# HKUST-KnowComp/DualMessagePassing

Measured on AMD Instinct MI355X. Metric: (pattern,graph) pairs/sec DMPNN fwd+bwd hid=128, higher is better.
Workload: dtype f32

## Files before the change

dualmessagepassing_amd/csrc/dmp_nodechain.hip:

```cpp
#include "dmp_mfma_common.h"

namespace dmp {
__device__ int llvm_struct_buffer_load_i32(i32x4 rsrc, int vindex, int voffset, int soffset, int aux) __asm("llvm.amdgcn.struct.buffer.load.i32");
__device__ void llvm_struct_buffer_store_i32(int data, i32x4 rsrc, int vindex, int voffset, int soffset, int aux) __asm("llvm.amdgcn.struct.buffer.store.i32");
namespace {

constexpr int kChainThreads = 512;
constexpr int kChainRows = 128;
constexpr int kChainStrideD = 68;
constexpr int kChainPlane = kChainRows * kChainStrideD;
constexpr int kChainImageBytes = 3 * kChainPlane * 4;
constexpr int kChainPanelBytes = 3 * 128 * 128 * 2;
constexpr int kChainChunkBytes = kChainPanelBytes / 4;
constexpr int kChainLdsBytes = kChainImageBytes + 2 * kChainChunkBytes + kChainRows * 4;
constexpr int kChainMaxPanels = 12;

__device__ __forceinline__ float sbuf_load1(srsrc_t r, int row, uint32_t col_bytes) {
  return __int_as_float(llvm_struct_buffer_load_i32(r, row, (int)col_bytes, 0, 0));
}
__device__ __forceinline__ void sbuf_store1(float v, srsrc_t r, int row, uint32_t col_bytes) {
  llvm_struct_buffer_store_i32(__float_as_int(v), r, row, (int)col_bytes, 0, 0);
}

struct PackArgs {
  const float *W[kChainMaxPanels];
  int64_t ld[kChainMaxPanels];
  int transposed[kChainMaxPanels];
  uint32_t *out;
};
__global__ __launch_bounds__(256) void chain_pack_k(PackArgs p) {
  const int item = (int)blockIdx.x * 256 + (int)threadIdx.x;
  const int lane = item & 63, cb = (item >> 6) & 3, g = item >> 8;
  const int li = lane & 31, h = lane >> 5;
  const float *W = nullptr;
  int64_t ld = 0;
  int tr = 0;
#pragma unroll
  for (int j = 0; j < kChainMaxPanels; ++j)
    if (j == (int)blockIdx.y) { W = p.W[j]; ld = p.ld[j]; tr = p.transposed[j]; }
  const int k0 = 64 * h + 8 * g, c = 32 * cb + li;
  float w[8];
#pragma unroll
  for (int j = 0; j < 8; ++j) w[j] = tr ? W[(int64_t)c * ld + k0 + j] : W[(int64_t)(k0 + j) * ld + c];
  Split8 s;
  split8(make_float4(w[0], w[1], w[2], w[3]), make_float4(w[4], w[5], w[6], w[7]), s);
  uint32_t *o = p.out + (size_t)blockIdx.y * (kChainPanelBytes / 4) + (size_t)g * 3072 + cb * 256 + lane * 4;
  *reinterpret_cast<uint4 *>(o) = make_uint4(s.hi.u[0], s.hi.u[1], s.hi.u[2], s.hi.u[3]);
  *reinterpret_cast<uint4 *>(o + 1024) = make_uint4(s.mid.u[0], s.mid.u[1], s.mid.u[2], s.mid.u[3]);
  *reinterpret_cast<uint4 *>(o + 2048) = make_uint4(s.lo.u[0], s.lo.u[1], s.lo.u[2], s.lo.u[3]);
}

struct ChainArgs {
  const float *A0, *A1, *A2;
  int64_t lda0, lda1, lda2;
  const float *X; int64_t ldx;
  const float *Res; int64_t ldres;
  const float *bias1, *bias2;
  float *O0, *O1, *O2, *O3;
  int64_t ldo0, ldo1, ldo2, ldo3;
  float *partial, *partialA;
  const uint32_t *panels;
  int npanels;
  const int32_t *slot; const int32_t *num_tiles;
  int64_t rows;
  float slope;
};

template <bool BWD, bool FULL>
__global__ __launch_bounds__(kChainThreads) void node_chain_k(ChainArgs p) {
  extern __shared__ __attribute__((aligned(256))) unsigned char lds[];
  uint32_t *Aimg = reinterpret_cast<uint32_t *>(lds);
  unsigned char *Pb = lds + kChainImageBytes;
  int *ids_s = reinterpret_cast<int *>(lds + kChainImageBytes + 2 * kChainChunkBytes);

  const int t = threadIdx.x;
  const int wave = __builtin_amdgcn_readfirstlane(t >> 6);
  const int lane = t & 63, li = lane & 31, h = lane >> 5;
  const int rt = wave >> 1, ch = wave & 1;
  const int q = t & 31, r0 = t >> 5;
  const float slope = __builtin_bit_cast(float, __builtin_amdgcn_readfirstlane(__builtin_bit_cast(int, p.slope)));
  const bool has_res = p.Res != nullptr;
  const int NC = __builtin_amdgcn_readfirstlane(p.npanels) * 4;
  constexpr bool full = FULL;

  const int ntiles = __builtin_amdgcn_readfirstlane(*p.num_tiles);
  const int chunk = (ntiles + (int)gridDim.x - 1) / (int)gridDim.x;
  const int lo = (int)blockIdx.x * chunk;
  const int hi = lo + chunk < ntiles ? lo + chunk : ntiles;
  if (hi <= lo) {
    if (BWD && t < 128) { p.partial[(int64_t)blockIdx.x * 128 + t] = 0.f; p.partialA[(int64_t)blockIdx.x * 128 + t] = 0.f; }
    return;
  }
  const rsrc_t rs_slot = make_rsrc(p.slot, (uint32_t)hi * (kSub * 4u));
  const rsrc_t rs_pan = make_rsrc(p.panels, (uint32_t)NC * (uint32_t)kChainChunkBytes);
  const srsrc_t rs_A0 = make_srsrc(p.A0, p.lda0, p.rows), rs_A1 = make_srsrc(p.A1, p.lda1, p.rows), rs_A2 = make_srsrc(p.A2, p.lda2, p.rows);
  const srsrc_t rs_X = make_srsrc(p.X, p.X ? p.ldx : (int64_t)128, p.X ? p.rows : 0);
  const srsrc_t rs_Res = make_srsrc(p.Res, has_res ? p.ldres : (int64_t)128, has_res ? p.rows : 0);
  const srsrc_t rs_O0 = make_srsrc(p.O0, p.ldo0, p.rows), rs_O1 = make_srsrc(p.O1, p.ldo1, p.rows), rs_O2 = make_srsrc(p.O2, p.ldo2, p.rows);
  const srsrc_t rs_O3 = make_srsrc(p.O3, p.O3 ? p.ldo3 : (int64_t)128, p.O3 ? p.rows : 0);

  int ids[8];
  float4 pre[8];
  auto load_ids = [&](int tile0) {
#pragma unroll
    for (int m = 0; m < 8; ++m) {
      const int idx = tile0 * kSub + r0 + 16 * m;
      const int v = (int)__builtin_amdgcn_raw_buffer_load_b32(rs_slot, idx * 4, 0, 0);
      ids[m] = idx < hi * kSub ? v : -1;
    }
  };
  auto load_rows = [&](srsrc_t rs) {
#pragma unroll
    for (int m = 0; m < 8; ++m) pre[m] = sbuf_load4(rs, ids[m], (uint32_t)q * 16u);
  };
  float4 csA = make_float4(0.f, 0.f, 0.f, 0.f);
  auto stage = [&](bool first) {
#pragma unroll
    for (int m = 0; m < 8; ++m) {
      const int row = r0 + 16 * m;
      if (BWD && first) { csA.x += pre[m].x; csA.y += pre[m].y; csA.z += pre[m].z; csA.w += pre[m].w; }
      uint2 ph, pm, pl;
      split_pair(pre[m].x, pre[m].y, ph.x, pm.x, pl.x);
      split_pair(pre[m].z, pre[m].w, ph.y, pm.y, pl.y);
      uint32_t *d = Aimg + row * kChainStrideD + q * 2;
      *reinterpret_cast<uint2 *>(d) = ph;
      *reinterpret_cast<uint2 *>(d + kChainPlane) = pm;
      *reinterpret_cast<uint2 *>(d + 2 * kChainPlane) = pl;
      if (first && q == 0) ids_s[row] = ids[m];
    }
  };

  f32x16 acc[2];
  auto zero_acc = [&]() {
#pragma unroll
    for (int r = 0; r < 16; ++r) { acc[0][r] = 0.f; acc[1][r] = 0.f; }
  };
  auto product = [&](int pidx) {
#pragma unroll
    for (int cc = 0; cc < 4; ++cc) {
      const int c = 4 * pidx + cc;
      const int nc = c + 1 == NC ? 0 : c + 1;
      uint4 pc[3];
#pragma unroll
      for (int i = 0; i < 3; ++i) {
        const u32x4 v = __builtin_amdgcn_raw_buffer_load_b128(rs_pan, (i * kChainThreads + t) * 16, nc * kChainChunkBytes, 0);
        pc[i] = make_uint4(v.x, v.y, v.z, v.w);
      }
      const unsigned char *pb = Pb + (cc & 1) * kChainChunkBytes;
      const uint32_t *ar = Aimg + (32 * rt + li) * kChainStrideD + 32 * h;
#pragma unroll
      for (int gl = 0; gl < 2; ++gl) {
        const int g = 2 * cc + gl;
        Split8 a;
        a.hi.v = *reinterpret_cast<const bf16x8 *>(ar + 4 * g);
        a.mid.v = *reinterpret_cast<const bf16x8 *>(ar + kChainPlane + 4 * g);
        a.lo.v = *reinterpret_cast<const bf16x8 *>(ar + 2 * kChainPlane + 4 * g);
#pragma unroll
        for (int cbl = 0; cbl < 2; ++cbl) {
          const unsigned char *bq = pb + gl * 12288 + (2 * ch + cbl) * 1024 + lane * 16;
          Split8 b;
          b.hi.v = *reinterpret_cast<const bf16x8 *>(bq);
          b.mid.v = *reinterpret_cast<const bf16x8 *>(bq + 4096);
          b.lo.v = *reinterpret_cast<const bf16x8 *>(bq + 8192);
          acc[cbl] = mfma_x6(a, b, acc[cbl]);
        }
      }
      uint4 *pw = reinterpret_cast<uint4 *>(Pb + ((cc + 1) & 1) * kChainChunkBytes);
#pragma unroll
      for (int i = 0; i < 3; ++i) pw[i * kChainThreads + t] = pc[i];
      lds_barrier();
    }
  };
  int rid[16];
  auto store_acc = [&](srsrc_t rs) {
#pragma unroll
    for (int cb = 0; cb < 2; ++cb)
#pragma unroll
      for (int r = 0; r < 16; ++r) sbuf_store1(acc[cb][r], rs, rid[r], (uint32_t)(64 * ch + 32 * cb + li) * 4u);
  };
  auto acc_to_image = [&]() {
#pragma unroll
    for (int cb = 0; cb < 2; ++cb)
#pragma unroll
      for (int i = 0; i < 8; ++i) {
        const float va = acc[cb][2 * i], vb = acc[cb][2 * i + 1];
        const float got = __shfl_xor((li & 1) ? va : vb, 1, 64);
        const float f0 = (li & 1) ? got : va, f1 = (li & 1) ? vb : got;
        const int r = 2 * i + (li & 1);
        const int row = 32 * rt + (r & 3) + 8 * (r >> 2) + 4 * h;
        uint32_t ph, pm, pl;
        split_pair(f0, f1, ph, pm, pl);
        uint32_t *d = Aimg + row * kChainStrideD + 32 * ch + 16 * cb + (li >> 1);
        d[0] = ph; d[kChainPlane] = pm; d[2 * kChainPlane] = pl;
      }
  };
  float colsum[2] = {0.f, 0.f};

  load_ids(lo);
  load_rows(rs_A0);
  {
    uint4 *pw = reinterpret_cast<uint4 *>(Pb);
#pragma unroll
    for (int i = 0; i < 3; ++i) {
      const u32x4 v = __builtin_amdgcn_raw_buffer_load_b128(rs_pan, (i * kChainThreads + t) * 16, 0, 0);
      pw[i * kChainThreads + t] = make_uint4(v.x, v.y, v.z, v.w);
    }
  }
  for (int g0 = lo; g0 < hi; g0 += 4) {
    stage(true);
    lds_barrier();
#pragma unroll
    for (int qd = 0; qd < 4; ++qd) {
      const int4 v = *reinterpret_cast<const int4 *>(&ids_s[32 * rt + 8 * qd + 4 * h]);
      rid[4 * qd] = v.x; rid[4 * qd + 1] = v.y; rid[4 * qd + 2] = v.z; rid[4 * qd + 3] = v.w;
    }
    if (!BWD) {
      load_rows(rs_A1);
      zero_acc(); product(0); store_acc(rs_O0);
      zero_acc(); product(1); store_acc(rs_O1);
      zero_acc(); product(2);
      stage(false); lds_barrier();
      load_rows(rs_A2);
      product(3);
      stage(false); lds_barrier();
      load_ids(g0 + 4);
      product(4);
      load_rows(rs_A0);
#pragma unroll
      for (int cb = 0; cb < 2; ++cb) {
        const float b = p.bias1[64 * ch + 32 * cb + li];
#pragma unroll
        for (int r = 0; r < 16; ++r) acc[cb][r] = act_fwd(acc[cb][r] + b, slope);
      }
      float res[2][16];
#pragma unroll
      for (int cb = 0; cb < 2; ++cb)
#pragma unroll
        for (int r = 0; r < 16; ++r) res[cb][r] = sbuf_load1(rs_Res, rid[r], (uint32_t)(64 * ch + 32 * cb + li) * 4u);
      store_acc(rs_O2);
      acc_to_image();
      lds_barrier();
      zero_acc(); product(5);
#pragma unroll
      for (int cb = 0; cb < 2; ++cb) {
        const float b = p.bias2[64 * ch + 32 * cb + li];
#pragma unroll
        for (int r = 0; r < 16; ++r) acc[cb][r] = res[cb][r] + (acc[cb][r] + b);
      }
      store_acc(rs_O3);
    } else {
      float hv[2][16];
#pragma unroll
      for (int cb = 0; cb < 2; ++cb)
#pragma unroll
        for (int r = 0; r < 16; ++r) hv[cb][r] = sbuf_load1(rs_X, rid[r], (uint32_t)(64 * ch + 32 * cb + li) * 4u);
      zero_acc(); product(0);
      if (full) load_rows(rs_A1);
      else load_ids(g0 + 4);
#pragma unroll
      for (int cb = 0; cb < 2; ++cb)
#pragma unroll
        for (int r = 0; r < 16; ++r) {
          acc[cb][r] = act_bwd(hv[cb][r], acc[cb][r], slope);
          colsum[cb] += acc[cb][r];
        }
      store_acc(rs_O0);
      acc_to_image();
      lds_barrier();
      zero_acc(); product(1);
      if (!full) load_rows(rs_A0);
      store_acc(rs_O1);
      zero_acc(); product(2); store_acc(rs_O2);
      if (full) {
        zero_acc(); product(3);
        stage(false); lds_barrier();
        load_rows(rs_A2);
        product(4);
        stage(false); lds_barrier();
        load_ids(g0 + 4);
        float res[2][16];
#pragma unroll
        for (int cb = 0; cb < 2; ++cb)
#pragma unroll
          for (int r = 0; r < 16; ++r) res[cb][r] = sbuf_load1(rs_Res, rid[r], (uint32_t)(64 * ch + 32 * cb + li) * 4u);
        product(5);
        load_rows(rs_A0);
#pragma unroll
        for (int cb = 0; cb < 2; ++cb)
#pragma unroll
          for (int r = 0; r < 16; ++r) acc[cb][r] = res[cb][r] + acc[cb][r];
        store_acc(rs_O3);
      }
    }
  }
  if (BWD) {
    float *red = reinterpret_cast<float *>(Pb);
    float *redA = red + 4 * 128;
#pragma unroll
    for (int cb = 0; cb < 2; ++cb) {
      const float s = colsum[cb] + __shfl_xor(colsum[cb], 32, 64);
      if (h == 0) red[rt * 128 + 64 * ch + 32 * cb + li] = s;
    }
    *reinterpret_cast<float4 *>(&redA[r0 * 128 + q * 4]) = csA;
    lds_barrier();
    if (t < 128) {
      float s = red[t];
#pragma unroll
      for (int w = 1; w < 4; ++w) s += red[w * 128 + t];
      p.partial[(int64_t)blockIdx.x * 128 + t] = s;
      float sa = redA[t];
#pragma unroll
      for (int w = 1; w < 16; ++w) sa += redA[w * 128 + t];
      p.partialA[(int64_t)blockIdx.x * 128 + t] = sa;
    }
  }
}

inline unsigned chain_blocks(int64_t tiles_bound) {
  const int64_t want = (tiles_bound + 3) / 4;
  return (unsigned)(want < 1 ? 1 : (want > 256 ? 256 : want));
}

constexpr int kMaxDevicesC = 64;
template <bool BWD, bool FULL>
inline bool chain_lds_ready() {
  static bool done[kMaxDevicesC] = {};
  int dev = 0;
  if (hipGetDevice(&dev) != hipSuccess || dev < 0 || dev >= kMaxDevicesC) dev = 0;
  if (done[dev]) return true;
  const hipError_t e = hipFuncSetAttribute(reinterpret_cast<const void *>(&node_chain_k<BWD, FULL>), hipFuncAttributeMaxDynamicSharedMemorySize, kChainLdsBytes);
  if (e != hipSuccess) { set_last_hip_error(e); return false; }
  done[dev] = true;
  return true;
}

inline bool chain_rows_ok(const float *a, int64_t ld, int64_t rows) {
  return a && ld >= 128 && ld % 4 == 0 && aligned16(a) && stride_ok(ld) && fits4g(rows, ld);
}

}
}

using namespace dmp;

extern "C" {

int64_t dmp_node_chain_blocks(int64_t tiles_bound) { return (int64_t)chain_blocks(tiles_bound); }
int64_t dmp_node_chain_panel_words(void) { return kChainPanelBytes / 4; }

int dmp_node_chain_pack(const dmp_chain_panel *panels, int num_panels, uint32_t *out, void *stream) {
  if (!panels || !out || num_panels < 1 || num_panels > kChainMaxPanels || !aligned16(out)) return DMP_ERR_BAD_ARG;
  PackArgs a{};
  for (int j = 0; j < num_panels; ++j) {
    if (!panels[j].W || panels[j].ld < 128) return DMP_ERR_BAD_ARG;
    a.W[j] = panels[j].W; a.ld[j] = panels[j].ld; a.transposed[j] = panels[j].transposed ? 1 : 0;
  }
  a.out = out;
  chain_pack_k<<<dim3(8, (unsigned)num_panels), 256, 0, (hipStream_t)stream>>>(a);
  return check_launch();
}

int dmp_node_chain_fwd(const float *x, int64_t ldx, const float *S, int64_t lds, const uint32_t *panels, const float *bn, const float *b2,
                       int residual, float slope, const int32_t *slot, const int32_t *num_tiles, int64_t tiles_bound, int64_t rows, int H,
                       float *H1n, int64_t ldh, float *P, int64_t ldp, float *xn, int64_t ldxn, void *stream) {
  if (H != 128 || g_exact_fp32) return DMP_ERR_UNSUPPORTED;
  if (rows < 0 || tiles_bound < 0) return DMP_ERR_BAD_ARG;
  if (!slope_ok(slope)) return DMP_ERR_UNSUPPORTED;
  if (rows == 0 || tiles_bound == 0) return DMP_OK;
  if (!panels || !bn || !b2 || !slot || !num_tiles || !aligned16(panels)) return DMP_ERR_BAD_ARG;
  if (!x || !S || !H1n || !P || !xn || ldx < H || lds < 2 * H || ldh < H || ldp < 2 * H || ldxn < H) return DMP_ERR_BAD_ARG;
  if (!chain_rows_ok(x, ldx, rows) || !chain_rows_ok(S, lds, rows) || !chain_rows_ok(H1n, ldh, rows) || !chain_rows_ok(P, ldp, rows) ||
      !chain_rows_ok(xn, ldxn, rows) || rows >= ((int64_t)1 << 30) || tiles_bound * kSub * 4 >= ((int64_t)1 << 32) - 8192)
    return DMP_ERR_UNSUPPORTED;
  if (!chain_lds_ready<false, true>()) return DMP_ERR_HIP;
  ChainArgs a{};
  a.A0 = x; a.lda0 = ldx; a.A1 = S; a.lda1 = lds; a.A2 = S + H; a.lda2 = lds;
  a.Res = residual ? x : nullptr; a.ldres = ldx; a.bias1 = bn; a.bias2 = b2;
  a.O0 = P; a.ldo0 = ldp; a.O1 = P + H; a.ldo1 = ldp; a.O2 = H1n; a.ldo2 = ldh; a.O3 = xn; a.ldo3 = ldxn;
  a.panels = panels; a.npanels = 6; a.slot = slot; a.num_tiles = num_tiles; a.rows = rows; a.slope = slope;
  node_chain_k<false, true><<<chain_blocks(tiles_bound), kChainThreads, kChainLdsBytes, (hipStream_t)stream>>>(a);
  return check_launch();
}

int dmp_node_chain_bwd(const float *dxn, int64_t ldd, const float *H1n, int64_t ldh, const float *dP, int64_t ldp, const uint32_t *panels,
                       int residual, float slope, const int32_t *slot, const int32_t *num_tiles, int64_t tiles_bound, int64_t rows, int H,
                       float *dPn, int64_t ldn, float *dS, int64_t lds, float *dx, int64_t ldx, float *partial, float *partial_rows,
                       void *stream) {
  if (H != 128 || g_exact_fp32) return DMP_ERR_UNSUPPORTED;
  if (rows < 0 || tiles_bound < 0) return DMP_ERR_BAD_ARG;
  if (!slope_ok(slope)) return DMP_ERR_UNSUPPORTED;
  if (!partial || !partial_rows) return DMP_ERR_BAD_ARG;
  hipStream_t st = (hipStream_t)stream;
  if (rows == 0 || tiles_bound == 0) {
    const size_t bytes = sizeof(float) * 128 * (size_t)chain_blocks(tiles_bound);
    if (hipMemsetAsync(partial, 0, bytes, st) != hipSuccess || hipMemsetAsync(partial_rows, 0, bytes, st) != hipSuccess) return DMP_ERR_HIP;
    return DMP_OK;
  }
  if (!panels || !slot || !num_tiles || !aligned16(panels)) return DMP_ERR_BAD_ARG;
  if (!dxn || !H1n || !dPn || !dS || ldd < H || ldh < H || ldn < H || lds < 2 * H || (dx && (!dP || ldp < 2 * H || ldx < H))) return DMP_ERR_BAD_ARG;
  if (!chain_rows_ok(dxn, ldd, rows) || !chain_rows_ok(H1n, ldh, rows) || !chain_rows_ok(dPn, ldn, rows) || !chain_rows_ok(dS, lds, rows) ||
      (dx && (!chain_rows_ok(dP, ldp, rows) || !chain_rows_ok(dx, ldx, rows))) || rows >= ((int64_t)1 << 30) ||
      tiles_bound * kSub * 4 >= ((int64_t)1 << 32) - 8192)
    return DMP_ERR_UNSUPPORTED;
  if (!(dx ? chain_lds_ready<true, true>() : chain_lds_ready<true, false>())) return DMP_ERR_HIP;
  ChainArgs a{};
  a.A0 = dxn; a.lda0 = ldd;
  a.A1 = dx ? dP : dxn; a.lda1 = dx ? ldp : ldd; a.A2 = dx ? dP + H : dxn; a.lda2 = a.lda1;
  a.X = H1n; a.ldx = ldh; a.Res = (dx && residual) ? dxn : nullptr; a.ldres = ldd;
  a.O0 = dPn; a.ldo0 = ldn; a.O1 = dS; a.ldo1 = lds; a.O2 = dS + H; a.ldo2 = lds; a.O3 = dx; a.ldo3 = ldx;
  a.partial = partial; a.partialA = partial_rows;
  a.panels = panels; a.npanels = dx ? 6 : 3; a.slot = slot; a.num_tiles = num_tiles; a.rows = rows; a.slope = slope;
  if (dx) node_chain_k<true, true><<<chain_blocks(tiles_bound), kChainThreads, kChainLdsBytes, st>>>(a);
  else node_chain_k<true, false><<<chain_blocks(tiles_bound), kChainThreads, kChainLdsBytes, st>>>(a);
  return check_launch();
}

}
```

Before: 489,600.

## Stream weight panels directly to LDS and overlap output stores with next product

Panel chunks are now fetched with buffer-load-to-LDS instead of going through registers and then being written to shared memory. Each GEMM product's output stores are deferred into the first chunk iteration of the following product, so global stores overlap MFMA work, with hand-tuned vmcnt waits. The LDS layout is reordered so the panel buffers come first and the activation image offset is made opaque to the compiler. This cuts register pressure and VGPR-to-LDS traffic, but depends on fragile manual waitcnt counts that could race if the store count assumption is wrong.

Result: no change. 494,200, median of 6 (+0.9%).

```diff
diff --git a/dualmessagepassing_amd/csrc/dmp_nodechain.hip b/dualmessagepassing_amd/csrc/dmp_nodechain.hip
--- a/dualmessagepassing_amd/csrc/dmp_nodechain.hip
+++ b/dualmessagepassing_amd/csrc/dmp_nodechain.hip
@@ -69,9 +69,11 @@
 template <bool BWD, bool FULL>
 __global__ __launch_bounds__(kChainThreads) void node_chain_k(ChainArgs p) {
   extern __shared__ __attribute__((aligned(256))) unsigned char lds[];
-  uint32_t *Aimg = reinterpret_cast<uint32_t *>(lds);
-  unsigned char *Pb = lds + kChainImageBytes;
-  int *ids_s = reinterpret_cast<int *>(lds + kChainImageBytes + 2 * kChainChunkBytes);
+  unsigned char *Pb = lds;
+  int *ids_s = reinterpret_cast<int *>(lds + 2 * kChainChunkBytes);
+  int img_at = 2 * kChainChunkBytes + kChainRows * 4;
+  asm("" : "+v"(img_at));
+  uint32_t *Aimg = reinterpret_cast<uint32_t *>(lds + img_at);
 
   const int t = threadIdx.x;
   const int wave = __builtin_amdgcn_readfirstlane(t >> 6);
@@ -135,17 +137,27 @@
 #pragma unroll
     for (int r = 0; r < 16; ++r) { acc[0][r] = 0.f; acc[1][r] = 0.f; }
   };
-  auto product = [&](int pidx) {
+  int rid[16];
+  auto store_acc = [&](srsrc_t rs) {
+#pragma unroll
+    for (int cb = 0; cb < 2; ++cb)
+#pragma unroll
+      for (int r = 0; r < 16; ++r) sbuf_store1(acc[cb][r], rs, rid[r], (uint32_t)(64 * ch + 32 * cb + li) * 4u);
+  };
+  auto request_quarter = [&](int nc, int b) {
+#pragma unroll
+    for (int i = 0; i < 3; ++i)
+      __builtin_amdgcn_raw_ptr_buffer_load_lds(rs_pan, (__attribute__((address_space(3))) void *)(Pb + b * kChainChunkBytes + i * (kChainThreads * 16) + wave * 1024),
+                                               16, (i * kChainThreads + t) * 16, nc * kChainChunkBytes, 0, 0);
+  };
+  auto product = [&](int pidx, const srsrc_t *out) {
 #pragma unroll
     for (int cc = 0; cc < 4; ++cc) {
       const int c = 4 * pidx + cc;
-      const int nc = c + 1 == NC ? 0 : c + 1;
-      uint4 pc[3];
-#pragma unroll
-      for (int i = 0; i < 3; ++i) {
-        const u32x4 v = __builtin_amdgcn_raw_buffer_load_b128(rs_pan, (i * kChainThreads + t) * 16, nc * kChainChunkBytes, 0);
-        pc[i] = make_uint4(v.x, v.y, v.z, v.w);
-      }
+      request_quarter(c + 1 == NC ? 0 : c + 1, (cc + 1) & 1);
+      __builtin_amdgcn_sched_barrier(0);
+      const bool stores = cc == 0 && out != nullptr;
+      if (stores) { store_acc(*out); zero_acc(); }
       const unsigned char *pb = Pb + (cc & 1) * kChainChunkBytes;
       const uint32_t *ar = Aimg + (32 * rt + li) * kChainStrideD + 32 * h;
 #pragma unroll
@@ -165,18 +177,11 @@
           acc[cbl] = mfma_x6(a, b, acc[cbl]);
         }
       }
-      uint4 *pw = reinterpret_cast<uint4 *>(Pb + ((cc + 1) & 1) * kChainChunkBytes);
-#pragma unroll
-      for (int i = 0; i < 3; ++i) pw[i * kChainThreads + t] = pc[i];
+      __builtin_amdgcn_sched_barrier(0);
+      if (stores) asm volatile("s_waitcnt vmcnt(32)" ::: "memory");
+      else asm volatile("s_waitcnt vmcnt(0)" ::: "memory");
       lds_barrier();
     }
-  };
-  int rid[16];
-  auto store_acc = [&](srsrc_t rs) {
-#pragma unroll
-    for (int cb = 0; cb < 2; ++cb)
-#pragma unroll
-      for (int r = 0; r < 16; ++r) sbuf_store1(acc[cb][r], rs, rid[r], (uint32_t)(64 * ch + 32 * cb + li) * 4u);
   };
   auto acc_to_image = [&]() {
 #pragma unroll
@@ -196,16 +201,10 @@
   };
   float colsum[2] = {0.f, 0.f};
 
+  request_quarter(0, 0);
   load_ids(lo);
   load_rows(rs_A0);
-  {
-    uint4 *pw = reinterpret_cast<uint4 *>(Pb);
-#pragma unroll
-    for (int i = 0; i < 3; ++i) {
-      const u32x4 v = __builtin_amdgcn_raw_buffer_load_b128(rs_pan, (i * kChainThreads + t) * 16, 0, 0);
-      pw[i * kChainThreads + t] = make_uint4(v.x, v.y, v.z, v.w);
-    }
-  }
+  asm volatile("s_waitcnt vmcnt(0)" ::: "memory");
   for (int g0 = lo; g0 < hi; g0 += 4) {
     stage(true);
     lds_barrier();
@@ -216,15 +215,15 @@
     }
     if (!BWD) {
       load_rows(rs_A1);
-      zero_acc(); product(0); store_acc(rs_O0);
-      zero_acc(); product(1); store_acc(rs_O1);
-      zero_acc(); product(2);
+      zero_acc(); product(0, nullptr);
+      product(1, &rs_O0);
+      product(2, &rs_O1);
       stage(false); lds_barrier();
       load_rows(rs_A2);
-      product(3);
+      product(3, nullptr);
       stage(false); lds_barrier();
       load_ids(g0 + 4);
-      product(4);
+      product(4, nullptr);
       load_rows(rs_A0);
 #pragma unroll
       for (int cb = 0; cb < 2; ++cb) {
@@ -237,10 +236,9 @@
       for (int cb = 0; cb < 2; ++cb)
 #pragma unroll
         for (int r = 0; r < 16; ++r) res[cb][r] = sbuf_load1(rs_Res, rid[r], (uint32_t)(64 * ch + 32 * cb + li) * 4u);
-      store_acc(rs_O2);
       acc_to_image();
       lds_barrier();
-      zero_acc(); product(5);
+      product(5, &rs_O2);
 #pragma unroll
       for (int cb = 0; cb < 2; ++cb) {
         const float b = p.bias2[64 * ch + 32 * cb + li];
@@ -254,7 +252,7 @@
       for (int cb = 0; cb < 2; ++cb)
 #pragma unroll
         for (int r = 0; r < 16; ++r) hv[cb][r] = sbuf_load1(rs_X, rid[r], (uint32_t)(64 * ch + 32 * cb + li) * 4u);
-      zero_acc(); product(0);
+      zero_acc(); product(0, nullptr);
       if (full) load_rows(rs_A1);
       else load_ids(g0 + 4);
 #pragma unroll
@@ -264,18 +262,17 @@
           acc[cb][r] = act_bwd(hv[cb][r], acc[cb][r], slope);
           colsum[cb] += acc[cb][r];
         }
-      store_acc(rs_O0);
       acc_to_image();
       lds_barrier();
-      zero_acc(); product(1);
+      product(1, &rs_O0);
       if (!full) load_rows(rs_A0);
-      store_acc(rs_O1);
-      zero_acc(); product(2); store_acc(rs_O2);
+      product(2, &rs_O1);
+      if (!full) store_acc(rs_O2);
       if (full) {
-        zero_acc(); product(3);
+        product(3, &rs_O2);
         stage(false); lds_barrier();
         load_rows(rs_A2);
-        product(4);
+        product(4, nullptr);
         stage(false); lds_barrier();
         load_ids(g0 + 4);
         float res[2][16];
@@ -283,7 +280,7 @@
         for (int cb = 0; cb < 2; ++cb)
 #pragma unroll
           for (int r = 0; r < 16; ++r) res[cb][r] = sbuf_load1(rs_Res, rid[r], (uint32_t)(64 * ch + 32 * cb + li) * 4u);
-        product(5);
+        product(5, nullptr);
         load_rows(rs_A0);
 #pragma unroll
         for (int cb = 0; cb < 2; ++cb)
```
